# chonlei/neural-ode-ion-channels

Measured on AMD Instinct MI355X. Metric: trajectories/sec (sinewave protocol, 100k steps), higher is better.
Workload: dtype f64

## Files before the change

neural-ode-ion-channels_amd/csrc/ionode_attempt_body.hpp:

```cpp
#ifdef IONODE_STAMPS
    constexpr int NET = std::is_same<typename std::decay<decltype(IONODE_NET)>::type, MlpShrink4>::value ? 1 : 0;
    const unsigned long long att0_ = stamp_now();
#endif
    if constexpr (LW) {
#pragma unroll
      for (int i = 0; i < NPAR; ++i) asm volatile("" : "+v"(p[i]));
    }
    bool failed_now = false;
    if (active) {
      if ((int64_t)since >= a.max_steps || (int64_t)nacc + nrej >= a.max_total) { status = IONODE_STATUS_MAX_STEPS; failed_now = true; }
      else if (!(t + dt > t)) { status = IONODE_STATUS_DT_UNDERFLOW; failed_now = true; }
      else {
        bool fin = true;
#pragma unroll
        for (int d = 0; d < D; ++d) fin = fin && isfinite((double)y[d]);
        if (!fin) { status = IONODE_STATUS_NONFINITE; failed_now = true; }
      }
      if (failed_now) active = false;
    }
    {
      unsigned long long fm = __ballot(failed_now && lane < LPS);
      while (fm) {
        const int jj = __builtin_ctzll(fm);
        fm &= fm - 1;
        if (WPS == 1 || (jj % WPS) == wis) {
          const int o0 = __builtin_amdgcn_readlane(oi, jj);
          const int tr = __builtin_amdgcn_readlane(traj, jj);
          S *__restrict__ yo = reinterpret_cast<S *>(a.y_out) + (size_t)tr * Nt * D;
          for (int idx = o0 + lane; idx < Nt && (a.y_out || a.i_out); idx += 64) {
            if (a.y_out) {
#pragma unroll
              for (int d = 0; d < D; ++d) yo[(size_t)idx * D + d] = nan_s;
            }
            if (a.i_out) a.i_out[(size_t)tr * Nt + idx] = __builtin_nan("");
          }
        }
      }
    }
    if constexpr (NSETS > 1) {
      if (__syncthreads_or(active ? 1 : 0) == 0) break;
    } else {
      if (__ballot(active) == 0ull) break;
    }

    const double t0 = t;
    const double t1 = t0 + dt;
    const S dts = (S)dt;
    S k[7][D], yi[D];
#pragma unroll
    for (int d = 0; d < D; ++d) k[0][d] = f[d];
    if constexpr (!CARRY_V) lookup_stages(t0, dt);
    STAMP(stamps_, 1);
    ClosedRates<MT::MLP ? IONODE_MODEL_HH2 : MODEL> cr;
#pragma unroll
    for (int i = 0; i < 6; ++i) {
      S bd[6];
#pragma unroll
      for (int jx = 0; jx <= i; ++jx) bd[jx] = (S)kBeta[i][jx] * dts;
#pragma unroll
      for (int d = 0; d < D; ++d) {
        S s = k[0][d] * bd[0];
#pragma unroll
        for (int jx = 1; jx <= i; ++jx) s = s + k[jx][d] * bd[jx];
        yi[d] = y[d] + s;
      }
      if constexpr (MT::MLP && T64) {
        bool fresh = (i == 0);
        if (i > 0 && i < 5) fresh = __ballot(vst[i] != vst[i > 0 ? i - 1 : 0] || inst[i] != inst[i > 0 ? i - 1 : 0]) != 0ull;
        rhs<MODEL, S, T64>(a, p, vst[i < 4 ? i : 4], inst[i < 4 ? i : 4], yi, k[i + 1], IONODE_NET, &cr, fresh);
      } else if constexpr (MT::MLP) rhs<MODEL, S, T64>(a, p, vst[i < 4 ? i : 4], inst[i < 4 ? i : 4], yi, k[i + 1], IONODE_NET);
      else {
        if (i < 5) {
          bool fresh = (i == 0);
          if (i > 0) fresh = __ballot(vst[i] != vst[i > 0 ? i - 1 : 0] || inst[i] != inst[i > 0 ? i - 1 : 0]) != 0ull;
          if (fresh) closed_rates<MODEL, S>(a, p, vst[i], inst[i], cr);
        }
        closed_rhs<MODEL, S>(cr, yi, k[i + 1]);
      }
    }
    S tmp[D];
    {
      S be[7];
#pragma unroll
      for (int jx = 0; jx < 7; ++jx) be[jx] = dts * (S)kCerr[jx];
#pragma unroll
      for (int d = 0; d < D; ++d) {
        S e = k[0][d] * be[0];
#pragma unroll
        for (int jx = 1; jx < 7; ++jx) e = e + k[jx][d] * be[jx];
        const S ay0 = abs_(y[d]), ay1 = abs_(yi[d]);
        const S tol = atol + rtol * (ay0 > ay1 ? ay0 : ay1);
        tmp[d] = e / tol;
      }
    }
    const S ratio = abs_(rms_norm<S, D>(tmp));
    const bool accept = ratio <= (S)1;

    double dt_next;
    if (ratio == (S)0) dt_next = dt * 10.0;
    else {
      const double dfactor = (ratio < (S)1) ? 1.0 : 0.2;
      const double er = (double)ratio;
      double fac = 0.9 / det_root5(er);
      if (!(fac > dfactor)) fac = dfactor;
      if (!(fac < 10.0)) fac = 10.0;
      if (er != er) fac = __builtin_nan("");
      dt_next = dt * fac;
    }

    STAMP(stamps_, 6);
    const bool acc_now = active && accept;
#ifndef IONODE_STAMPS
    if (a.step_log != nullptr && active && primary && traj_raw == 0 && (int64_t)nacc + nrej < a.step_log_cap) {
      double *row = a.step_log + 4 * ((int64_t)nacc + nrej);
      row[0] = t0; row[1] = dt; row[2] = (double)ratio; row[3] = accept ? 1.0 : 0.0;
    }
#endif
    const int nacc_before = nacc, oi_before = oi;
    if (active) { if (accept) ++nacc; else ++nrej; }
    const double dt_capped = (dt_next > a.dt_max) ? a.dt_max : dt_next;
    if constexpr (CARRY_V) lookup_stages(acc_now ? t1 : t0, (active || acc_now) ? dt_capped : dt);

    const double den = t1 - t0;
    const double rden = 1.0 / den;
    constexpr int ROW = 4 + 5 * D;
    S ic[LW ? 1 : 5][LW ? 1 : D];
    {
      S bm[7];
#pragma unroll
      for (int jx = 0; jx < 7; ++jx) bm[jx] = dts * (S)kCmid[jx];
      auto fit = [&](int d, S *c5) {
        S s = k[0][d] * bm[0];
#pragma unroll
        for (int jx = 1; jx < 7; ++jx) s = s + k[jx][d] * bm[jx];
        const S YM = y[d] + s;
        const S F0 = k[0][d], F1 = k[6][d], Y0 = y[d], Y1 = yi[d];
        c5[4] = ((S)2 * dts) * (F1 - F0) - (S)8 * (Y1 + Y0) + (S)16 * YM;
        c5[3] = dts * ((S)5 * F0 - (S)3 * F1) + (S)18 * Y0 + (S)14 * Y1 - (S)32 * YM;
        c5[2] = dts * (F1 - (S)4 * F0) - (S)11 * Y0 - (S)5 * Y1 + (S)16 * YM;
        c5[1] = dts * F0;
        c5[0] = Y0;
      };
      if constexpr (LW) {
        double2 *row = reinterpret_cast<double2 *>(lsm + lane * ROWB);
        row[0] = make_double2(t0, den);
        row[1] = make_double2(rden, 0.0);
        static_assert(D % 2 == 0, "rows hold component pairs");
#pragma unroll
        for (int d = 0; d < D; d += 2) {
          S ca[5], cb2[5];
          fit(d, ca);
          fit(d + 1, cb2);
#pragma unroll
          for (int c = 0; c < 5; ++c) row[2 + (c * D + d) / 2] = make_double2((double)ca[c], (double)cb2[c]);
          if constexpr (D > 2) __builtin_amdgcn_sched_barrier(0);
        }
      } else {
#pragma unroll
        for (int d = 0; d < D; ++d) {
          S c5[5];
          fit(d, c5);
#pragma unroll
          for (int c = 0; c < 5; ++c) ic[c][d] = c5[c];
        }
      }
    }
    STAMP(stamps_, 8);
    if (LEAN || LEANM || a.te_dt > 0.0) {
      int n_out = 0;
      if (acc_now) {
        const double gf = floor((t1 - a.te_t0) * a.te_rdt);
        long long g = (gf < (double)(oi - 1)) ? (long long)(oi - 1) : ((gf > (double)(Nt - 1)) ? (long long)(Nt - 1) : (long long)gf);
        if ((LW && LEAN && D > 2) || (!LW && a.te_exact)) {
          while (g >= oi && te_at((int)g) > t1) --g;
          while (g + 1 < Nt && te_at((int)g + 1) <= t1) ++g;
        } else {
          while (g >= oi && a.t_eval[g] > t1) --g;
          while (g + 1 < Nt && a.t_eval[g + 1] <= t1) ++g;
        }
        n_out = (int)(g - oi + 1);
      }
      STAMP(stamps_, 9);
      if constexpr (!LW && G > 1) {
      constexpr int NS = (LPS >= WPS) ? LPS / WPS : 1;
      const bool exact = a.te_exact != 0;
      const bool want_i = (a.i_out != nullptr) || (a.sse_out != nullptr);
      const bool ugrid = a.prot_t == nullptr;
      int o_[NS], n_[NS], ip_[NS];
      double tk_[NS], plo_[NS], phi_[NS];
      bool inr_[NS];
      const double *pv_[NS];
#pragma unroll
      for (int k = 0; k < NS; ++k) {
        const int jj = wis + WPS * k;
        o_[k] = __builtin_amdgcn_readlane(oi, jj);
        n_[k] = (LPS >= WPS || jj < LPS) ? __builtin_amdgcn_readlane(n_out, jj) : 0;
        pv_[k] = a.prot_v + (size_t)__builtin_amdgcn_readlane(pidx, jj) * a.Np;
        tk_[k] = 0.0;
        if (lane < n_[k]) tk_[k] = exact ? te_at(o_[k] + lane) : a.t_eval[o_[k] + lane];
      }
      if (want_i && ugrid) {
#pragma unroll
        for (int k = 0; k < NS; ++k) {
          inr_[k] = protocol_index(a, tk_[k], ip_[k]);
          plo_[k] = pv_[k][ip_[k] - 1]; phi_[k] = pv_[k][ip_[k]];
        }
      }
      STAMP(stamps_, 10);
#pragma unroll
      for (int k = 0; k < NS; ++k) {
        const int jj = wis + WPS * k;
        const int n = n_[k], o = o_[k];
        if (n > 0) {
          const double t0b = bcast_f64(t0, jj), denb = bcast_f64(den, jj), rdenb = bcast_f64(rden, jj);
          S cb[5][D];
#pragma unroll
          for (int c = 0; c < 5; ++c)
#pragma unroll
            for (int d = 0; d < D; ++d) cb[c][d] = bcast<S>(ic[c][d], jj);
          const int tr = __builtin_amdgcn_readlane(traj, jj);
          S *__restrict__ yo = a.y_out ? reinterpret_cast<S *>(a.y_out) + (size_t)tr * Nt * D : nullptr;
          double *__restrict__ io = a.i_out ? a.i_out + (size_t)tr * Nt : nullptr;
          const double *__restrict__ refb = a.sse_out ? a.sse_ref + (size_t)__builtin_amdgcn_readlane(pidx, jj) * Nt : nullptr;
          double sacc = 0.0;
          for (int c0 = 0; c0 < n; c0 += 64) {
            const int idx = o + c0 + lane;
            double tk = tk_[k];
            if (c0 > 0 && c0 + lane < n) tk = exact ? te_at(idx) : a.t_eval[idx];
            if (c0 + lane < n) {
              const S x = (S)div_pos(tk - t0b, denb, rdenb);
              S out[D];
              S xp = x;
#pragma unroll
              for (int d = 0; d < D; ++d) out[d] = cb[0][d] + x * cb[1][d];
#pragma unroll
              for (int c = 2; c < 5; ++c) {
                xp = xp * x;
#pragma unroll
                for (int d = 0; d < D; ++d) out[d] = out[d] + xp * cb[c][d];
              }
              if (yo) store_state<S, D>(yo + (size_t)idx * D, out);
              if (want_i) {
                double vk;
                if (c0 == 0 && ugrid) vk = inr_[k] ? protocol_from(a, plo_[k], phi_[k], ip_[k], tk) : a.v_oob;
                else protocol_v(a, pv_[k], tk, vk);
                S gate;
                if (a.obs_open) gate = out[D - 1]; else gate = out[0] * out[1];
                if (a.obs_g != 1.0) gate = (S)a.obs_g * gate;
                const double ik = (double)gate * (vk - a.obs_e);
                if (io) io[idx] = ik;
                if (refb) { const double rr = ik - refb[idx]; sacc += rr * rr; }
              }
            }
          }
          if (a.sse_out) {
#pragma unroll
            for (int msk = 32; msk >= 1; msk >>= 1) sacc += __shfl_xor(sacc, msk);
            if (j == jj) sse += sacc;
          }
        }
      }
      oi += n_out;
      } else {
      bool packed_lane = false;
      if constexpr (LW && (VTAB || D > 2 || (CF2 && TAIL == 1))) {
#ifndef IONODE_PACK_PKL_D6
#define IONODE_PACK_PKL_D6 2
#endif
        constexpr int PK = 8, PKL = (D == 2) ? 4 : IONODE_PACK_PKL_D6, NSL = PK / PKL;
        typedef S SV __attribute__((ext_vector_type(NSL)));
        const bool want_i = (a.i_out != nullptr) || (a.sse_out != nullptr);
        if (a.te_exact && (VTAB ? (want_i && (D > 2 || a.y_out == nullptr)) : (!want_i && a.y_out != nullptr))) {
          int lane_e = lane;
          asm volatile("" : "+v"(lane_e));
          packed_lane = n_out > 0 && lane_e < LPS && n_out <= 64;
          const unsigned long long emd = __ballot(packed_lane);
          auto emit_packed = [&](auto wi_tag) {
            constexpr bool WI = decltype(wi_tag)::value;
            const int nch = (n_out + PK - 1) / PK;
            if (packed_lane) *reinterpret_cast<int2 *>(lsm + lane_e * ROWB + 24) = make_int2(oi, oi + n_out);
            const int x = nch - 1;
            const unsigned long long m0 = __ballot(packed_lane && (x & 1)), m1 = __ballot(packed_lane && (x & 2)), m2 = __ballot(packed_lane && (x & 4));
            const int q = mbcnt(m0, mbcnt(emd)) + 2 * mbcnt(m1) + 4 * mbcnt(m2);
            const int C = __builtin_popcountll(emd) + __builtin_popcountll(m0) + 2 * __builtin_popcountll(m1) + 4 * __builtin_popcountll(m2);
#pragma unroll
            for (int i = 0; i < 8; ++i)
              if (packed_lane && i < nch) clist[q + i] = (unsigned short)(lane_e | (i * PK) << 6);
            const int slot = lane_e / PKL, kk = lane_e % PKL;
            struct Ent { int jj, idx0, end, part; bool has; double vk[NSL], rf[NSL]; };
            auto decode = [&](int c0) {
              Ent t;
              t.has = c0 + slot < C;
              const unsigned e = clist[t.has ? c0 + slot : (c0 < C ? c0 : 0)];
              t.jj = (int)(e & 63u);
              t.part = (int)(e >> 9);
              const int2 on2 = *reinterpret_cast<const int2 *>(lsm + t.jj * ROWB + 24);
              t.idx0 = on2.x + (int)(e >> 6) + kk;
              t.end = on2.y;
#pragma unroll
              for (int u = 0; u < NSL; ++u) { t.vk[u] = 0.0; t.rf[u] = 0.0; }
              if constexpr (VTAB && WI) {
                const int pj = owp[t.jj];
#pragma unroll
                for (int u = 0; u < NSL; ++u) {
                  const int idx = t.idx0 + u * PKL;
                  if (t.has && idx < t.end) {
                    t.vk[u] = a.v_tab[(size_t)pj * Nt + idx];
                    if (a.sse_out) t.rf[u] = a.sse_ref[(size_t)pj * Nt + idx];
                  }
                }
              }
              return t;
            };
            constexpr bool PREF = (D > 2);
            Ent nx{};
            if constexpr (PREF) nx = decode(0);
            for (int c0 = 0; c0 < C; c0 += 64 / PKL) {
              const Ent cur = PREF ? nx : decode(c0);
              if constexpr (PREF) { if (c0 + 64 / PKL < C) nx = decode(c0 + 64 / PKL); }
              const int jj = cur.jj;
              const double2 *rj = reinterpret_cast<const double2 *>(lsm + jj * ROWB);
              const double2 h0 = rj[0];
              const double t0b = h0.x, denb = h0.y, rdenb = rj[1].x;
              S cb[5][D];
#pragma unroll
              for (int c = 0; c < 5; ++c)
#pragma unroll
                for (int d = 0; d < D; d += 2) {
                  const double2 cc = rj[2 + (c * D + d) / 2];
                  cb[c][d] = (S)cc.x; cb[c][d + 1] = (S)cc.y;
                }
              const int tr = trl[jj];
              double tk[NSL];
              SV xv;
#pragma unroll
              for (int u = 0; u < NSL; ++u) {
                tk[u] = te_at(cur.idx0 + u * PKL);
                xv[u] = (S)div_pos(tk[u] - t0b, denb, rdenb);
              }
              SV ov[D], xp = xv;
#pragma unroll
              for (int d = 0; d < D; ++d) ov[d] = cb[0][d] + xv * cb[1][d];
#pragma unroll
              for (int c = 2; c < 5; ++c) {
                xp = xp * xv;
#pragma unroll
                for (int d = 0; d < D; ++d) ov[d] = ov[d] + xp * cb[c][d];
              }
              double rr2[NSL];
#pragma unroll
              for (int u = 0; u < NSL; ++u) {
                const int idx = cur.idx0 + u * PKL;
                rr2[u] = 0.0;
                if (cur.has && idx < cur.end) {
                  S out[D];
#pragma unroll
                  for (int d = 0; d < D; ++d) out[d] = ov[d][u];
                  if (!WI || a.y_out) store_state<S, D>(reinterpret_cast<S *>(a.y_out) + ((size_t)tr * Nt + idx) * D, out);
                  if constexpr (WI) {
                    double vk;
                    if constexpr (VTAB) vk = cur.vk[u];
                    else protocol_v(a, a.prot_v + (size_t)owp[jj] * a.Np, tk[u], vk);
                    S gate;
                    if (a.obs_open) gate = out[D - 1]; else gate = out[0] * out[1];
                    if (a.obs_g != 1.0) gate = (S)a.obs_g * gate;
                    const double ik = (double)gate * (vk - a.obs_e);
                    if (a.i_out) a.i_out[(size_t)tr * Nt + idx] = ik;
                    if (a.sse_out) { const double rr = ik - (VTAB ? cur.rf[u] : a.sse_ref[(size_t)owp[jj] * Nt + idx]); rr2[u] = rr * rr; }
                  }
                }
              }
              if (WI && a.sse_out) {
                double g8;
                if constexpr (PKL == 4) {
                  double ql = rr2[0] + dpp_f64<0xB1, 0xf>(rr2[0]), qh = rr2[1] + dpp_f64<0xB1, 0xf>(rr2[1]);
                  ql = ql + dpp_f64<0x4E, 0xf>(ql); qh = qh + dpp_f64<0x4E, 0xf>(qh);
                  g8 = ql + qh;
                } else {
                  double sj[NSL];
#pragma unroll
                  for (int u = 0; u < NSL; ++u) sj[u] = rr2[u] + dpp_f64<0xB1, 0xf>(rr2[u]);
                  g8 = (sj[0] + sj[1]) + (sj[2] + sj[3]);
                }
                if (kk == 0 && cur.has) ssep[jj * 8 + cur.part] += g8;
              }
            }
          };
          if (emd) emit_packed(std::integral_constant<bool, VTAB>{});
        }
      }
      {
      unsigned long long em = __ballot(n_out > 0 && lane < LPS && !packed_lane);
      if (G > 1) {
        unsigned long long mine = 0ull;
#pragma unroll
        for (int k = 0; k < (TPW + G - 1) / G; ++k) mine |= 1ull << (wave + k * G);
        em &= mine;
      }
      int jj = em ? __builtin_ctzll(em) : 0;
      int o = __builtin_amdgcn_readlane(oi, jj);
      const bool arith_t = LW && a.te_exact;
      double tk_nxt = (em && o + lane < Nt) ? (arith_t ? te_at(o + lane) : a.t_eval[o + lane]) : 0.0;
      double vk_nxt = 0.0, rf_nxt = 0.0;
      auto prefetch_obs = [&](int jx, int ox) {
        if constexpr (VTAB) {
          const int pjx = __builtin_amdgcn_readlane(pidx, jx);
          if (ox + lane < Nt) {
            vk_nxt = a.v_tab[(size_t)pjx * Nt + ox + lane];
            if (a.sse_out) rf_nxt = a.sse_ref[(size_t)pjx * Nt + ox + lane];
          }
        }
      };
      if (em) prefetch_obs(jj, o);
      while (em) {
        em &= em - 1;
        const int jn = em ? __builtin_ctzll(em) : 0;
        const int on = __builtin_amdgcn_readlane(oi, jn);
        double tk = tk_nxt;
        const double vk_first = vk_nxt, rf_first = rf_nxt;
        if (em && on + lane < Nt) tk_nxt = arith_t ? te_at(on + lane) : a.t_eval[on + lane];
        if (em) prefetch_obs(jn, on);
        const int n = __builtin_amdgcn_readlane(n_out, jj);
        double t0b, denb, rdenb;
        S cb[5][D];
        if constexpr (LW) {
          const double2 *rj = reinterpret_cast<const double2 *>(lsm) + jj * (ROW / 2);
          const double2 h0 = rj[0], h1 = rj[1];
          t0b = h0.x; denb = h0.y; rdenb = h1.x;
#pragma unroll
          for (int c = 0; c < 5; ++c)
#pragma unroll
            for (int d = 0; d < D; d += 2) {
              const double2 cc = rj[2 + (c * D + d) / 2];
              cb[c][d] = (S)cc.x; cb[c][d + 1] = (S)cc.y;
            }
        } else {
          t0b = bcast_f64(t0, jj); denb = bcast_f64(den, jj); rdenb = bcast_f64(rden, jj);
#pragma unroll
          for (int c = 0; c < 5; ++c)
#pragma unroll
            for (int d = 0; d < D; ++d) cb[c][d] = bcast<S>(ic[c][d], jj);
        }
        const int tr = __builtin_amdgcn_readlane(traj, jj);
        S *__restrict__ yo = a.y_out ? reinterpret_cast<S *>(a.y_out) + (size_t)tr * Nt * D : nullptr;
        double *__restrict__ io = nullptr;
        const double *__restrict__ pvb = nullptr, *__restrict__ refb = nullptr, *__restrict__ vtb = nullptr;
        if (a.i_out || a.sse_out) {
          if (a.i_out) io = a.i_out + (size_t)tr * Nt;
          int pj;
          if constexpr (LW) pj = __builtin_amdgcn_readlane(pidx, jj);
          else pj = a.prot_of_traj ? a.prot_of_traj[tr] : (tr % a.P);
          pvb = a.prot_v + (size_t)pj * a.Np;
          if (a.sse_out) refb = a.sse_ref + (size_t)pj * Nt;
          if constexpr (VTAB) vtb = a.v_tab + (size_t)pj * Nt;
        }
        double sacc = 0.0;
        for (int c0 = 0; c0 < n; c0 += 64) {
          const int idx = o + c0 + lane;
          if (c0 > 0 && c0 + lane < n) tk = arith_t ? te_at(idx) : a.t_eval[idx];
          if (c0 + lane < n) {
            const S x = (S)div_pos(tk - t0b, denb, rdenb);
            S out[D];
            S xp = x;
#pragma unroll
            for (int d = 0; d < D; ++d) out[d] = cb[0][d] + x * cb[1][d];
#pragma unroll
            for (int c = 2; c < 5; ++c) {
              xp = xp * x;
#pragma unroll
              for (int d = 0; d < D; ++d) out[d] = out[d] + xp * cb[c][d];
            }
            if (yo) store_state<S, D>(yo + (size_t)idx * D, out);
            if (pvb) {
              double vk;
              if constexpr (VTAB) vk = (c0 == 0) ? vk_first : vtb[idx];
              else protocol_v(a, pvb, tk, vk);
              S gate;
              if (a.obs_open) gate = out[D - 1]; else gate = out[0] * out[1];
              if (a.obs_g != 1.0) gate = (S)a.obs_g * gate;
              const double ik = (double)gate * (vk - a.obs_e);
              if (io) io[idx] = ik;
              if (refb) { const double rr = ik - ((VTAB && c0 == 0) ? rf_first : refb[idx]); sacc += rr * rr; }
            }
          }
        }
        if (a.sse_out) {
          if constexpr (LW) {
            const double g8 = group8_sum_f64(sacc);
            if ((lane & 7) == 0) ssep[jj * 8 + (lane >> 3)] += g8;
          } else {
#pragma unroll
            for (int msk = 32; msk >= 1; msk >>= 1) sacc += __shfl_xor(sacc, msk);
            if (j == jj) sse += sacc;
          }
        }
        jj = jn;
        o = on;
      }
      oi += n_out;
      }
      }
    } else {
      unsigned long long em = __ballot(acc_now && lane < LPS);
      while (em) {
        const int jj = __builtin_ctzll(em);
        em &= em - 1;
        const bool owner = (WPS == 1) || ((jj % WPS) == wis);
        int o = __builtin_amdgcn_readlane(oi, jj);
        const double t1b = bcast_f64(t1, jj);
        double t0b = 0.0, denb = 1.0, rdenb = 1.0;
        S cb[5][D];
        S *__restrict__ yo = nullptr;
        double *__restrict__ io = nullptr;
        const double *__restrict__ pvb = nullptr;
        if (owner) {
          if constexpr (LW) {
            const double2 *rj = reinterpret_cast<const double2 *>(lsm) + jj * (ROW / 2);
            const double2 h0 = rj[0], h1 = rj[1];
            t0b = h0.x; denb = h0.y; rdenb = h1.x;
#pragma unroll
            for (int c = 0; c < 5; ++c)
#pragma unroll
              for (int d = 0; d < D; d += 2) {
                const double2 cc = rj[2 + (c * D + d) / 2];
                cb[c][d] = (S)cc.x; cb[c][d + 1] = (S)cc.y;
              }
          } else {
            t0b = bcast_f64(t0, jj); denb = bcast_f64(den, jj); rdenb = bcast_f64(rden, jj);
#pragma unroll
            for (int c = 0; c < 5; ++c)
#pragma unroll
              for (int d = 0; d < D; ++d) cb[c][d] = bcast<S>(ic[c][d], jj);
          }
          const int tr = __builtin_amdgcn_readlane(traj, jj);
          yo = reinterpret_cast<S *>(a.y_out) + (size_t)tr * Nt * D;
          if (a.i_out) {
            io = a.i_out + (size_t)tr * Nt;
            const int pj = a.prot_of_traj ? a.prot_of_traj[tr] : (tr % a.P);
            pvb = a.prot_v + (size_t)pj * a.Np;
          }
        }
        for (;;) {
          const int idx = o + lane;
          const double tk = (idx < Nt) ? a.t_eval[idx] : __builtin_inf();
          const bool ok = tk <= t1b;
          if (owner && ok) {
            const S x = (S)div_pos(tk - t0b, denb, rdenb);
            S out[D];
            S xp = x;
#pragma unroll
            for (int d = 0; d < D; ++d) out[d] = cb[0][d] + x * cb[1][d];
#pragma unroll
            for (int c = 2; c < 5; ++c) {
              xp = xp * x;
#pragma unroll
              for (int d = 0; d < D; ++d) out[d] = out[d] + xp * cb[c][d];
            }
            store_state<S, D>(yo + (size_t)idx * D, out);
            if (io) {
              double vk;
              protocol_v(a, pvb, tk, vk);
              S gate;
              if (a.obs_open) gate = out[D - 1]; else gate = out[0] * out[1];
// ... 35 lines not shown
```

neural-ode-ion-channels_amd/csrc/ionode_device.hpp:

```cpp
#pragma once

#include <hip/hip_runtime.h>
#include <stdint.h>

#include <type_traits>

#include "../../include/ionode.h"

namespace ionode {

using f32x4 = __attribute__((ext_vector_type(4))) float;

struct KArgs {
  const float *mlp;
  const double *params;
  const double *prot_v;
  const double *prot_t;
  const int32_t *prot_of_traj;
  const void *y0;
  const double *t_eval;
  void *y_out;
  double *i_out;
  int32_t *status;
  int64_t *stats;
// ... 1473 lines not shown
    } else {
#pragma unroll
      for (int i = 0; i < NR; ++i) R.k[i] = p[2 * i] * det_exp_ldexp(x[i]);
    }
  }
}
template <int MODEL, typename S>
__device__ __forceinline__ void closed_rhs(const ClosedRates<MODEL> &R, const S *y, S *f) {
  if constexpr (MODEL == IONODE_MODEL_MARKOV6) {
    if (R.oob32) {
      const float a1 = R.kf[0], b1 = R.kf[1], bh = R.kf[2], ah = R.kf[3], a2 = R.kf[4], b2 = R.kf[5];
      const float c1 = y[0], c2 = y[1], i_ = y[2], ic1 = y[3], ic2 = y[4], o = y[5];
      f[0] = a1 * c2 + ah * ic1 + b2 * o - (b1 + bh + a2) * c1;
      f[1] = b1 * c1 + ah * ic2 - (a1 + bh) * c2;
      f[2] = a2 * ic1 + bh * o - (b2 + ah) * i_;
      f[3] = a1 * ic2 + bh * c1 + b2 * i_ - (b1 + ah + a2) * ic1;
      f[4] = b1 * ic1 + bh * c2 - (ah + a1) * ic2;
      f[5] = a2 * c1 + ah * i_ - (b2 + bh) * o;
      return;
    }
    const double a1 = R.k[0], b1 = R.k[1], bh = R.k[2], ah = R.k[3], a2 = R.k[4], b2 = R.k[5];
    const double c1 = y[0], c2 = y[1], i_ = y[2], ic1 = y[3], ic2 = y[4], o = y[5];
    f[0] = (S)(a1 * c2 + ah * ic1 + b2 * o - (b1 + bh + a2) * c1);
    f[1] = (S)(b1 * c1 + ah * ic2 - (a1 + bh) * c2);
    f[2] = (S)(a2 * ic1 + bh * o - (b2 + ah) * i_);
    f[3] = (S)(a1 * ic2 + bh * c1 + b2 * i_ - (b1 + ah + a2) * ic1);
    f[4] = (S)(b1 * ic1 + bh * c2 - (ah + a1) * ic2);
    f[5] = (S)(a2 * c1 + ah * i_ - (b2 + bh) * o);
  } else {
    const S av = y[0], rv = y[1];
    if (R.oob32) {
      const float af = (float)av, rf = (float)rv;
      const float drdt = -R.kf[2] * rf + R.kf[3] * (1.0f - rf);
      const float dadt = R.kf[0] * (1.0f - af) - R.kf[1] * af;
      f[0] = (S)dadt;
      f[1] = (S)drdt;
      return;
    }
    const S one_m_a = (S)1 - av, one_m_r = (S)1 - rv;
    const double drdt = -R.k[2] * (double)rv + R.k[3] * (double)one_m_r;
    const double dadt = R.k[0] * (double)one_m_a - R.k[1] * (double)av;
    f[0] = (S)dadt;
    f[1] = (S)drdt;
  }
}

template <typename S, int D> __device__ __forceinline__ S rms_norm(const S *x) {
  S s = x[0] * x[0];
#pragma unroll
  for (int i = 1; i < D; ++i) s = s + x[i] * x[i];
  s = s / (S)D;
  return Real<S>::sqrt_(s);
}
template <typename S> __device__ __forceinline__ S abs_(S x) { return x < 0 ? -x : x; }

#ifndef IONODE_M6_WAVES
#define IONODE_M6_WAVES 1
#endif
#ifndef IONODE_CF_WAVES
#ifndef IONODE_HH2_WAVES
#define IONODE_HH2_WAVES 2
#endif
#define IONODE_CF_WAVES(MODEL, G) ((G) > 1 ? 1 : ((MODEL) == IONODE_MODEL_HH2 ? IONODE_HH2_WAVES : IONODE_M6_WAVES))
#endif
#ifndef IONODE_T64_WAVES
#define IONODE_T64_WAVES 1
#endif
#ifndef IONODE_N100_WAVES
#define IONODE_N100_WAVES 1
#endif
#define IONODE_WAVES_PER_SIMD(MODEL, G, NT, RT) \
  (((MODEL) >= IONODE_MODEL_NNF && (RT) == 64) ? IONODE_T64_WAVES : (((MODEL) >= IONODE_MODEL_NNF && (NT) == 7) ? IONODE_N100_WAVES : IONODE_CF_WAVES(MODEL, G)))

template <typename S, int D> __device__ __forceinline__ void store_state(S *dst, const S *v) {
  if constexpr (D == 2 && sizeof(S) == 8) {
    *reinterpret_cast<double2 *>(dst) = make_double2(v[0], v[1]);
  } else if constexpr (D == 2 && sizeof(S) == 4) {
    *reinterpret_cast<float2 *>(dst) = make_float2(v[0], v[1]);
  } else if constexpr (sizeof(S) == 8) {
#pragma unroll
    for (int d = 0; d < D; d += 2) *reinterpret_cast<double2 *>(dst + d) = make_double2(v[d], v[d + 1]);
  } else {
#pragma unroll
    for (int d = 0; d < D; d += 2) *reinterpret_cast<float2 *>(dst + d) = make_float2(v[d], v[d + 1]);
  }
}

#define IONODE_LW_TILES_PER_WG 4
#define IONODE_IS_LW(MODEL, RT) ((MODEL) == IONODE_MODEL_HH2 || (MODEL) == IONODE_MODEL_MARKOV6 || (RT) == 64)
template <int MODEL, typename S, int G, int RT, int NT, int PD, int TAIL>
__global__ void __launch_bounds__(64 * (IONODE_IS_LW(MODEL, RT) ? IONODE_LW_TILES_PER_WG : G), IONODE_WAVES_PER_SIMD(MODEL, G, NT, RT)) ionode_dopri5_kernel(const KArgs a_in) {
  using MT = ModelTraits<MODEL>;
  constexpr bool LEAN = IONODE_LEAN && (!MT::MLP || RT == 64) && TAIL == 1;
  constexpr bool LEANT = IONODE_LEAN && !MT::MLP && TAIL == 2;
  constexpr bool LEANM = IONODE_LEAN && MT::MLP && G > 1 && (TAIL & 8);
  KArgs a = a_in;
  if constexpr (LEANM) a.te_exact = 1;
  if constexpr (LEAN || LEANT || LEANM) { a.prot_t = nullptr; a.step_log = nullptr; a.step_log_cap = 0; a.ckpt = nullptr; a.ckpt_cap = 0; }
  if constexpr (LEAN) { a.i_out = nullptr; a.sse_out = nullptr; a.sse_ref = nullptr; a.v_tab = nullptr; a.te_exact = 1; }
#ifdef IONODE_STAMPS
  a.step_log = a_in.step_log; a.step_log_cap = a_in.step_log_cap;
#endif
  using R = Real<S>;
  constexpr int D = MT::D, NPAR = MT::NPAR;
  constexpr bool T64 = MT::MLP && RT == 64;
  static_assert(!T64 || (G == 1 && NT == 1), "64 trajectories per wavefront is the resident-weights (N <= 16) path");
  constexpr bool LW = !MT::MLP || T64;
  constexpr int NSETS = (MT::MLP && G > 1 && (TAIL & 4)) ? 2 : 1;
  constexpr int WPS = G / NSETS;
  constexpr bool T4 = MT::MLP && G == 4 && NT == 13 && (TAIL & 16);
  static_assert(!T4 || NSETS == 1, "the 4-trajectory tile has one column set");
  constexpr bool T1 = MT::MLP && G == 4 && NT == 13 && (TAIL & 32);
  static_assert(!T1 || (NSETS == 1 && !T4), "the one-trajectory tile has one column set and is not the 4-trajectory tile");
  constexpr int TPW = MT::MLP ? (T64 ? 64 : (T1 ? 1 : (T4 ? 4 : 16 * NSETS))) : (RT > 0 ? RT : 64);
  constexpr int LPS = (MT::MLP && !T64) ? (T1 ? 1 : (T4 ? 4 : 16)) : TPW;
  static_assert(MT::MLP || G == 1, "closed-form models use one wavefront per tile");

  extern __shared__ __attribute__((aligned(16))) unsigned char smem[];

  const int lane = threadIdx.x & 63;
  const int wgw = __builtin_amdgcn_readfirstlane(threadIdx.x >> 6);
  const int wave = LW ? 0 : wgw;
  const int tile = LW ? (int)((blockIdx.x & 7u) + 8u * ((blockIdx.x >> 3) * (unsigned)IONODE_LW_TILES_PER_WG + (unsigned)wgw)) : (int)blockIdx.x;
  unsigned char *const smem_t = LW ? smem + (size_t)wgw * (size_t)a.lw_bytes : smem;
  if constexpr (LW) {
    if (tile * (MT::MLP ? 64 : (RT > 0 ? RT : 64)) >= a_in.B) return;
  }
  const int j = lane % LPS;
  const int cset = (NSETS > 1) ? wave / WPS : 0, wis = wave % WPS;
  const bool primary = (lane < LPS) && (wis == 0);
  const int slot_raw = tile * TPW + cset * LPS + j;
  const bool valid = slot_raw < a.B;
  const int slot_c = valid ? slot_raw : a.B - 1;
  const int traj = a.order ? a.order[slot_c] : slot_c;
  const int traj_raw = valid ? traj : a.B;

  constexpr bool VNET = T64 && PD > 1;
  constexpr bool GEN = MT::MLP && G == 4 && NT == 0;
  using MlpTileT = MlpTile<G, (T64 ? 1 : (RT > 0 ? RT : 1)), (NT > 0 ? NT : 1), ((PD > 0 && !VNET) ? PD : 1), (NSETS > 1 ? 4 : 0)>;
  using MlpT = typename std::conditional<VNET, MlpLane<(VNET ? PD : 10)>, typename std::conditional<T1, typename std::conditional<(TAIL & 64) != 0, MlpRow1Deep, MlpRow1>::type, typename std::conditional<T4, MlpTile4, typename std::conditional<GEN, MlpGen, MlpTileT>::type>::type>::type>::type;
  typename std::conditional<MT::MLP, MlpT, NoMlp>::type mlp;
  if constexpr (MT::MLP) mlp.init(a, smem_t, wave, lane, tile * TPW);
  size_t lw_off = 0;
  if constexpr (T64) lw_off = (MlpT::lds_bytes(a.L) + 15) & ~(size_t)15;
  unsigned char *const lsm = smem_t + lw_off;
  STAMP_DECL
#ifdef IONODE_STAMPS
  if constexpr (MT::MLP) mlp.sp = &stamps_;
#endif

  double p[NPAR];
#pragma unroll
  for (int i = 0; i < NPAR; ++i) p[i] = a.params[(size_t)traj * a.n_params + i];
  const int pidx = a.prot_of_traj ? a.prot_of_traj[traj] : (traj % a.P);
  const double *__restrict__ pv = a.prot_v + (size_t)pidx * a.Np;

  const S rtol = (S)a.rtol, atol = (S)a.atol;
  S *__restrict__ yout = reinterpret_cast<S *>(a.y_out) + (size_t)traj * a.Nt * D;
  double *__restrict__ iout = a.i_out ? a.i_out + (size_t)traj * a.Nt : nullptr;
  const int Nt = a.Nt;

  S y[D], f[D];
#pragma unroll
  for (int d = 0; d < D; ++d) y[d] = reinterpret_cast<const S *>(a.y0)[(size_t)traj * D + d];

  double t = a.t_eval[0];
  {
    double v0;
    const bool in0 = protocol_v(a, pv, (double)(S)t, v0);
    rhs<MODEL, S, T64>(a, p, v0, in0, y, f, mlp);
  }

  double dt;
  {
    const S t0s = (S)t;
    S scale[D], tmp[D], y1[D], f1[D];
#pragma unroll
    for (int d = 0; d < D; ++d) scale[d] = atol + abs_(y[d]) * rtol;
#pragma unroll
    for (int d = 0; d < D; ++d) tmp[d] = y[d] / scale[d];
    const S d0 = rms_norm<S, D>(tmp);
#pragma unroll
    for (int d = 0; d < D; ++d) tmp[d] = f[d] / scale[d];
    const S d1 = rms_norm<S, D>(tmp);
    S h0;
    if (d0 < (S)1e-5 || d1 < (S)1e-5) h0 = (S)1e-6;
    else h0 = (S)0.01 * d0 / d1;
#pragma unroll
    for (int d = 0; d < D; ++d) y1[d] = y[d] + h0 * f[d];
    {
      double v1;
      const bool in1 = protocol_v(a, pv, (double)(t0s + h0), v1);
      rhs<MODEL, S, T64>(a, p, v1, in1, y1, f1, mlp);
    }
#pragma unroll
    for (int d = 0; d < D; ++d) tmp[d] = (f1[d] - f[d]) / scale[d];
    const S d2 = rms_norm<S, D>(tmp) / h0;
    S h1;
    if (d1 <= (S)1e-15 && d2 <= (S)1e-15) {
      const S c = h0 * (S)1e-3;
      h1 = (S)1e-6 > c ? (S)1e-6 : c;
    } else {
      h1 = (S)det_root5((double)((S)0.01 / (d1 > d2 ? d1 : d2)));
    }
    const S h = ((S)100 * h0 < h1) ? (S)100 * h0 : h1;
    dt = (double)h;
    if (dt > a.dt_max) dt = a.dt_max;
  }

  constexpr bool CF2 = LW && D == 2;
  constexpr int LT = MT::MLP ? (TAIL == 1 ? 1 : 0) : TAIL;
  constexpr int ROWB = LwLds::rowb(D);
  constexpr bool VTAB = !MT::MLP && TAIL == 2;
  double *const ssep = reinterpret_cast<double *>(lsm + LwLds::aux_off(D));
  if constexpr (LW) {
    if (a.sse_out != nullptr) {
#pragma unroll
      for (int m = 0; m < 8; ++m) ssep[lane * 8 + m] = 0.0;
    }
  }
  int *const owp = reinterpret_cast<int *>(lsm + LwLds::owp_off(D, LT));
  int *const trl = reinterpret_cast<int *>(lsm + LwLds::trl_off(D, LT));
  unsigned short *const clist = reinterpret_cast<unsigned short *>(lsm + LwLds::clist_off(D, LT));
  if constexpr (LW) {
    if (lane < LPS) trl[lane] = traj, owp[lane] = pidx;
  }
  auto te_at = [&](int idx) -> double { return a.te_t0 + (double)idx * a.te_dt; };

  double sse = 0.0;
  if (valid && primary) {
    if (a.y_out) store_state<S, D>(yout, y);
    if (iout) {
      double v0;
      protocol_v(a, pv, t, v0);
      S gate;
      if (a.obs_open) gate = y[D - 1]; else gate = y[0] * y[1];
      if (a.obs_g != 1.0) gate = (S)a.obs_g * gate;
      iout[0] = (double)gate * (v0 - a.obs_e);
    }
  }
  if (a.sse_out != nullptr && valid) {
    double v0;
    protocol_v(a, pv, t, v0);
    S gate;
    if (a.obs_open) gate = y[D - 1]; else gate = y[0] * y[1];
    if (a.obs_g != 1.0) gate = (S)a.obs_g * gate;
    const double r0 = (double)gate * (v0 - a.obs_e) - a.sse_ref[(size_t)pidx * Nt];
    sse = r0 * r0;
  }

  int oi = 1;
  int nacc = 0, nrej = 0;
  int since = 0;
  int status = IONODE_STATUS_OK;
  bool active = valid && Nt > 1;
  const S nan_s = (S)__builtin_nan("");

  double vst[5];
  bool inst[5];
  auto lookup_stages = [&](double tt, double dd) {
    const S tts = (S)tt, dds = (S)dd, tt1s = (S)(tt + dd);
#ifndef IONODE_BATCH_LOOKUPS_ALL
#define IONODE_BATCH_LOOKUPS_ALL 0
#endif
#ifndef IONODE_BATCH_LOOKUPS_T64
#define IONODE_BATCH_LOOKUPS_T64 0
#endif
#ifndef IONODE_BATCH_LOOKUPS_CF
#define IONODE_BATCH_LOOKUPS_CF 1
#endif
    if (((MT::MLP && G > 1) || (IONODE_BATCH_LOOKUPS_CF && !MT::MLP && (D > 2 || TAIL != 2)) || (IONODE_BATCH_LOOKUPS_T64 && T64) || IONODE_BATCH_LOOKUPS_ALL) && a.prot_t == nullptr) {
      double tq[5], lo[5], hi[5];
      int ix[5];
#pragma unroll
      for (int i = 0; i < 5; ++i) {
        tq[i] = (double)((i >= 4) ? R::prev_(tt1s) : tts + (S)kAlpha[i] * dds);
        inst[i] = protocol_index(a, tq[i], ix[i]);
      }
#pragma unroll
      for (int i = 0; i < 5; ++i) { lo[i] = pv[ix[i] - 1]; hi[i] = pv[ix[i]]; }
#pragma unroll
      for (int i = 0; i < 5; ++i) vst[i] = inst[i] ? protocol_from(a, lo[i], hi[i], ix[i], tq[i]) : a.v_oob;
      return;
    }
#pragma unroll
    for (int i = 0; i < 5; ++i) {
      const S ti = (i >= 4) ? R::prev_(tt1s) : tts + (S)kAlpha[i] * dds;
      inst[i] = protocol_v(a, pv, (double)ti, vst[i]);
    }
  };
#ifndef IONODE_CARRY_V_TINY16
#define IONODE_CARRY_V_TINY16 1
#endif
#ifndef IONODE_CARRY_V_MLP
#define IONODE_CARRY_V_MLP 0
#endif
#ifndef IONODE_CARRY_V_M6
#define IONODE_CARRY_V_M6 1
#endif
  constexpr bool CARRY_V = (LW && D == 2) || (IONODE_CARRY_V_M6 && LW && D > 2 && LEAN) || (MT::MLP && (IONODE_CARRY_V_MLP || (IONODE_CARRY_V_TINY16 && G == 1)));
  if constexpr (CARRY_V) lookup_stages(t, dt);

  constexpr bool SHRINK = MT::MLP && G == 4 && NT == 13 && PD == 13 && TAIL == 8 && std::is_same<MlpT, MlpTileT>::value;
#ifdef IONODE_STAMPS
  unsigned long long att_cyc[2] = {0, 0}, att_n[2] = {0, 0};
#endif

  auto live_slots = [&]() { return (unsigned)__ballot(active) & 0xffffu; };
  bool more = true;
  if (!SHRINK || !a.tile_shrink || __builtin_popcount(live_slots()) > 4) {
    more = false;
    for (;;) {
#define IONODE_NET mlp
#include "ionode_attempt_body.hpp"
#undef IONODE_NET
      if constexpr (SHRINK) {
        if (a.tile_shrink && __builtin_popcount(live_slots()) <= 4) { more = true; break; }
      }
    }
  }
  if constexpr (SHRINK) {
    const unsigned live = live_slots();
    if (more && live != 0u) {
      asm volatile("s_waitcnt vmcnt(0) lgkmcnt(0)" ::: "memory");
      __syncthreads();
      MlpShrink4 net4;
      net4.init(a, smem_t, wave, lane, tile * TPW, live);
#ifdef IONODE_STAMPS
      net4.t4.sp = &stamps_;
#endif
      for (;;) {
#define IONODE_NET net4
#include "ionode_attempt_body.hpp"
#undef IONODE_NET
      }
    }
  }

#ifdef IONODE_STAMPS
  STAMP(stamps_, 0);
  if (blockIdx.x == 0 && threadIdx.x == 0 && a.step_log != nullptr && a.step_log_cap >= 4)
    for (int i_ = 0; i_ < 16; ++i_) a.step_log[i_] = (double)stamps_.acc[i_];
  if (threadIdx.x == 0 && a.step_log != nullptr) {
    if (blockIdx.x == 0 && a.step_log_cap >= 9) {
      a.step_log[32] = (double)att_cyc[0]; a.step_log[33] = (double)att_n[0];
      a.step_log[34] = (double)att_cyc[1]; a.step_log[35] = (double)att_n[1];
    }
    if (4 * a.step_log_cap >= 64 + (int64_t)gridDim.x) a.step_log[64 + blockIdx.x] = (double)att_n[1];
  }
#ifdef IONODE_ASM_STAMPS
  if constexpr (MT::MLP && G == 4 && NT == 13) {
    unsigned sv_;
    asm volatile("v_accvgpr_read_b32 %0, a92" : "=v"(sv_));
    if (blockIdx.x == 0 && threadIdx.x < 16 && a.step_log != nullptr && a.step_log_cap >= 8) a.step_log[16 + threadIdx.x] = (double)sv_;
  }
#endif
#endif
  if constexpr (LW) {
    if (a.sse_out != nullptr) {
#pragma unroll
      for (int m = 0; m < 8; ++m) sse += ssep[j * 8 + m];
    }
  }
  if (a.sse_out != nullptr && valid && lane < LPS && (WPS == 1 || (lane % WPS) == wis))
    a.sse_out[traj] = (status == IONODE_STATUS_OK) ? sse : __builtin_inf();
  if (valid && primary) {
    a.status[traj] = status;
    if (a.stats) {
      int64_t *st = a.stats + (size_t)traj * 4;
      st[0] = nacc;
      st[1] = nrej;
      st[2] = 2 + 6 * ((int64_t)nacc + nrej);
      st[3] = status;
    }
  }
}

}
```

Measured before the change: 12420.

## Pack dense-output emission across four tile trajectories into full wavefront lanes

In the tiled MLP path (SHRINK configuration), dense-output points from the four trajectories owned by a wavefront are compacted into a single prefix-summed index space. All 64 lanes then evaluate interpolants and currents together, using ds_bpermute to fetch each owning trajectory's coefficients and times. The next chunk's protocol lookup is software-prefetched while the current one is processed. This is meant to remove the lane underutilisation of the per-trajectory emit loop, at the cost of many cross-lane permutes per chunk. The path is skipped when SSE accumulation is requested.

```diff
diff --git a/neural-ode-ion-channels_amd/csrc/ionode_attempt_body.hpp b/neural-ode-ion-channels_amd/csrc/ionode_attempt_body.hpp
--- a/neural-ode-ion-channels_amd/csrc/ionode_attempt_body.hpp
+++ b/neural-ode-ion-channels_amd/csrc/ionode_attempt_body.hpp
@@ -186,6 +186,81 @@
       const bool exact = a.te_exact != 0;
       const bool want_i = (a.i_out != nullptr) || (a.sse_out != nullptr);
       const bool ugrid = a.prot_t == nullptr;
+      bool packed_tile = false;
+      if constexpr (TPACK) {
+        if (a.sse_out == nullptr) {
+          packed_tile = true;
+          static_assert(NS == 4 && LPS == 16 && WPS == 4, "four owned trajectories per wavefront, one per 16-lane row of the layout");
+          int lane_e = lane;
+          asm volatile("" : "+v"(lane_e));
+          const int n0 = __builtin_amdgcn_readlane(n_out, wis), n1 = __builtin_amdgcn_readlane(n_out, wis + WPS);
+          const int n2 = __builtin_amdgcn_readlane(n_out, wis + 2 * WPS), n3 = __builtin_amdgcn_readlane(n_out, wis + 3 * WPS);
+          const int c1 = n0, c2 = c1 + n1, c3 = c2 + n2, tot = c3 + n3;
+          auto perm_i = [&](int src4, int v) -> int { return __builtin_amdgcn_ds_bpermute(src4, v); };
+          auto perm_d = [&](int src4, double v) -> double {
+            return __hiloint2double(perm_i(src4, __double2hiint(v)), perm_i(src4, __double2loint(v)));
+          };
+          auto perm_s = [&](int src4, S v) -> S {
+            if constexpr (sizeof(S) == 8) return perm_d(src4, v);
+            else return __int_as_float(perm_i(src4, __float_as_int(v)));
+          };
+          struct Pk { int src4, idx, ip; bool has, inr; double tk, plo, phi; };
+          auto prep = [&](int f0) {
+            Pk q;
+            const int fl = f0 + lane_e;
+            const int kq = (fl >= c1 ? 1 : 0) + (fl >= c2 ? 1 : 0) + (fl >= c3 ? 1 : 0);
+            const int first = (kq == 0) ? 0 : ((kq == 1) ? c1 : ((kq == 2) ? c2 : c3));
+            q.src4 = ((lane_e & 48) | (wis + WPS * kq)) << 2;
+            q.has = fl < tot;
+            q.idx = perm_i(q.src4, oi) + (fl - first);
+            q.tk = q.has ? te_at(q.idx) : 0.0;
+            q.ip = 1; q.inr = false; q.plo = 0.0; q.phi = 0.0;
+            if (want_i) {
+              const double *__restrict__ pvq = a.prot_v + (size_t)perm_i(q.src4, pidx) * a.Np;
+              q.inr = protocol_index(a, q.tk, q.ip);
+              q.plo = pvq[q.ip - 1]; q.phi = pvq[q.ip];
+            }
+            return q;
+          };
+          Pk nx = prep(0);
+          STAMP(stamps_, 10);
+          for (int f0 = 0; f0 < tot; f0 += 64) {
+            const Pk cur = nx;
+            if (f0 + 64 < tot) nx = prep(f0 + 64);
+            const double t0b = perm_d(cur.src4, t0), denb = perm_d(cur.src4, den), rdenb = perm_d(cur.src4, rden);
+            S cb[5][D];
+#pragma unroll
+            for (int c = 0; c < 5; ++c)
+#pragma unroll
+              for (int d = 0; d < D; ++d) cb[c][d] = perm_s(cur.src4, ic[c][d]);
+            const int tr = perm_i(cur.src4, traj);
+            if (cur.has) {
+              const int idx = cur.idx;
+              const double tk = cur.tk;
+              const S x = (S)div_pos(tk - t0b, denb, rdenb);
+              S out[D];
+              S xp = x;
+#pragma unroll
+              for (int d = 0; d < D; ++d) out[d] = cb[0][d] + x * cb[1][d];
+#pragma unroll
+              for (int c = 2; c < 5; ++c) {
+                xp = xp * x;
+#pragma unroll
+                for (int d = 0; d < D; ++d) out[d] = out[d] + xp * cb[c][d];
+              }
+              if (a.y_out) store_state<S, D>(reinterpret_cast<S *>(a.y_out) + ((size_t)tr * Nt + idx) * D, out);
+              if (a.i_out) {
+                const double vk = cur.inr ? protocol_from(a, cur.plo, cur.phi, cur.ip, tk) : a.v_oob;
+                S gate;
+                if (a.obs_open) gate = out[D - 1]; else gate = out[0] * out[1];
+                if (a.obs_g != 1.0) gate = (S)a.obs_g * gate;
+                a.i_out[(size_t)tr * Nt + idx] = (double)gate * (vk - a.obs_e);
+              }
+            }
+          }
+        }
+      }
+      if (!packed_tile) {
       int o_[NS], n_[NS], ip_[NS];
       double tk_[NS], plo_[NS], phi_[NS];
       bool inr_[NS];
@@ -259,6 +334,7 @@
             if (j == jj) sse += sacc;
           }
         }
+      }
       }
       oi += n_out;
       } else {
diff --git a/neural-ode-ion-channels_amd/csrc/ionode_device.hpp b/neural-ode-ion-channels_amd/csrc/ionode_device.hpp
--- a/neural-ode-ion-channels_amd/csrc/ionode_device.hpp
+++ b/neural-ode-ion-channels_amd/csrc/ionode_device.hpp
@@ -1799,6 +1799,10 @@
   if constexpr (CARRY_V) lookup_stages(t, dt);
 
   constexpr bool SHRINK = MT::MLP && G == 4 && NT == 13 && PD == 13 && TAIL == 8 && std::is_same<MlpT, MlpTileT>::value;
+#ifndef IONODE_TILE_EMIT_PACKED
+#define IONODE_TILE_EMIT_PACKED 1
+#endif
+  constexpr bool TPACK = IONODE_TILE_EMIT_PACKED && SHRINK;
 #ifdef IONODE_STAMPS
   unsigned long long att_cyc[2] = {0, 0}, att_n[2] = {0, 0};
 #endif
```

Result: faster. 12550, median of 6 (+1.0%).
